# laurits-mumberg/kube-scheduler-simulator-p9

Hardware: AMD Instinct MI355X
Metric: filter+score pod x node pairs/sec (5k nodes, Fit+BalancedAllocation) (higher is better)
Workload: dtype int64+f64; 1 GPU; cfg2: 5,000 nodes x 10,000 pods, NodeResourcesFit+NodeResourcesBalancedAllocation; nodes_per_gpu=5000, nodes_total=5000, pods=10000, parallelism=1 GPU

## Files before the change

kube-scheduler-simulator-p9_amd/csrc/engine.hip:

```cpp
#include <hip/hip_runtime.h>

#include <algorithm>
#include <cmath>
#include <cstdlib>
#include <cstring>
#include <memory>
#include <string>
#include <vector>
#include <utility>
#include <deque>
#include <atomic>
#include <map>
#include <mutex>
#include <chrono>
#include <cstddef>
#include <thread>

#include "engine.h"
#include <rccl/rccl.h>

namespace ksg {

#define HIPCHK(x)                                                                 \
  do {                                                                            \
// ... 3319 lines not shown
    if (c == 0) {
      sm->feasible = feas;
      if (feas) {
        if (pt >= 0) {
          sm->max_score[pt] = max(red[0][0], red[1][0]) > sm->max_score[pt] ? max(red[0][0], red[1][0]) : sm->max_score[pt];
          sm->min_score[pt] = min(red[0][1], red[1][1]) < sm->min_score[pt] ? min(red[0][1], red[1][1]) : sm->min_score[pt];
        }
        if (pa >= 0) {
          sm->max_score[pa] = max(red[0][2], red[1][2]) > sm->max_score[pa] ? max(red[0][2], red[1][2]) : sm->max_score[pa];
          sm->min_score[pa] = min(red[0][3], red[1][3]) < sm->min_score[pa] ? min(red[0][3], red[1][3]) : sm->min_score[pa];
        }
      }
    }
    if (phase == 1) {
      A.wc_cls[(size_t)j * KSG_WC_CLS + c] = m;
      if (c == 0) A.wc_flag[j] = flag;
      return;
    }
    __syncthreads();
  } else {
    flag = A.wc_flag[j];
  }
  const bool kept = A.keep_n && q >= A.keep_first && q < A.keep_first + A.keep_n;
  if (kept) return;
  const int32_t feas_all = sm->feasible;
  const int64_t Mt = pt >= 0 ? sm->max_score[pt] : 0, Ma = pa >= 0 ? sm->max_score[pa] : 0;
  const int64_t wt = pt >= 0 ? F.weight[pt] : 0, wa = pa >= 0 ? F.weight[pa] : 0;
  bool range_err = false;
  uint64_t best = 0;
  if (present) {
    int64_t tot = (int64_t)(m >> 40);
    if (pt >= 0) {
      const int64_t s = Mt == 0 ? 100 : 100 - 100 * xt / Mt;
      range_err |= s < 0 || s > 100;
      tot += s * wt;
    }
    if (pa >= 0 && !(h->flags & KPF_SKIP_NA_SCORE)) {
      const int64_t s = Ma == 0 ? xa : 100 * xa / Ma;
      range_err |= s < 0 || s > 100;
      tot += s * wa;
    }
    if (feas_all == 1) tot = 0;
    best = ((uint64_t)tot << 40) | (m & 0xFFFFFFFFFFull);
  }
  best = wave_max(best);
  range_err = __ballot(range_err) != 0;
  if (lane == 0) {
    red[w][4] = (int64_t)best;
    red[w][5] = range_err ? 1 : 0;
  }
  __syncthreads();
  if (c == 0) {
    const uint64_t b = (uint64_t)red[0][4] > (uint64_t)red[1][4] ? (uint64_t)red[0][4] : (uint64_t)red[1][4];
    if (b) atomicMax((unsigned long long*)&sm->best_key, (unsigned long long)b);
    if (feas_all > 1 && (flag || red[0][5] || red[1][5])) atomicOr((uint32_t*)&sm->status, 2u);
  }
}

__device__ __forceinline__ int pend_index(int32_t gid, int32_t pn, int np) {
  int hit = -1;
  for (int e = 0; e < np; ++e) hit = __builtin_amdgcn_readlane(pn, e) == gid ? e : hit;
  return hit;
}
__device__ __forceinline__ void lds_barrier() { asm volatile("s_waitcnt lgkmcnt(0)\n\ts_barrier" ::: "memory"); }
__device__ __forceinline__ uint64_t ld_agent(const uint64_t* p) {
  return __hip_atomic_load(p, __ATOMIC_RELAXED, __HIP_MEMORY_SCOPE_AGENT);
}

struct PatchV {
  uint32_t code;
  int32_t fitba;
  int32_t total;
  uint32_t raw;
};
struct ShallowRows {
  RowV row[KSG_STAGE];
};
__device__ __forceinline__ ShallowRows* shallow_rows(uint8_t* rec) { return reinterpret_cast<ShallowRows*>(rec_rows(rec)); }
__device__ __forceinline__ const ShallowRows* shallow_rows(const uint8_t* rec) {
  return reinterpret_cast<const ShallowRows*>(rec_rows(rec));
}
static_assert(KSG_BATCH * sizeof(ShallowRows) <= kRecKeys * sizeof(RowV), "shallow rows fit the rows area");
static_assert(sizeof(ShallowRows) % 8 == 0, "8-byte words");
template <bool PER>
__device__ __forceinline__ void win_merge(const DevCluster& C, const WinArgs& A, uint32_t b, uint64_t* L, const int32_t* pnl,
                                          int np) {
  const int lane = threadIdx.x & 63, w = threadIdx.x >> 6;
  auto pend_lds = [&](int32_t gid) {
    int hit = -1;
    for (int e = 0; e < np; ++e) hit = pnl[e] == gid ? e : hit;
    return hit;
  };
  int32_t f[3] = {0, 0, 0};
  {
    const uint64_t* src = A.tile_top + (size_t)b * A.T * KSG_TOPK;
    uint64_t v = 0;
    if ((uint32_t)w < A.T) v = ld_agent(src + (size_t)w * KSG_TOPK + lane);
    if (w == 0)
      for (uint32_t t = lane; t < A.T; t += 64)
#pragma unroll
        for (int k = 0; k < 3; ++k)
          f[k] += __hip_atomic_load(A.tile_feas + ((size_t)b * A.T + t) * 3 + k, __ATOMIC_RELAXED, __HIP_MEMORY_SCOPE_AGENT);
#pragma unroll 1
    for (uint32_t t = w + 16; t < A.T; t += 16) v = wave_merge_top(v, ld_agent(src + (size_t)t * KSG_TOPK + 63 - lane));
    L[w * 64 + lane] = v;
  }
  lds_barrier();
  int s0 = 1;
  while (s0 < (int)A.T && s0 < 16) s0 <<= 1;
#pragma unroll 1
  for (int s = s0 >> 1; s >= 1; s >>= 1) {
    if (w < s) L[w * 64 + lane] = wave_merge_top(L[w * 64 + lane], L[(w + s) * 64 + 63 - lane]);
    lds_barrier();
  }
  if (w == 0) {
    const uint64_t v = L[lane];
    const int32_t gid = (int32_t)(v & 0xFFFFFull);
    stv<PER>(rec_keys(A.erec) + (size_t)b * KSG_CAND + lane, v);
    if (PER ? lane < KSG_STAGE : !A.xrows) {
      RowV c;
      memset(&c, 0, sizeof(c));
      if (v) {
        const int hh = pend_lds(gid);
        if (hh >= 0) c = ld_obj<PER>(&A.pprev[hh].after);
        else load_row_p<PER>(C, (uint32_t)gid - C.goff, A.need_eph, c);
      }
      st_obj<PER>(PER ? &shallow_rows(A.erec)[b].row[lane] : rec_rows(A.erec) + (size_t)b * KSG_CAND + lane, c);
    }
#pragma unroll
    for (int k = 0; k < 3; ++k) f[k] = wave_sum(f[k]);
    if (lane == 0) {
#pragma unroll
      for (int k = 0; k < 3; ++k) stv<PER>(reinterpret_cast<int32_t*>(A.erec) + k * KSG_BATCH + b, f[k]);
      stv<PER>(A.arrive + b * A.astride, 0u);
    }
    if constexpr (PER) {
      asm volatile("s_waitcnt vmcnt(0)" ::: "memory");
      if (lane == 0) __hip_atomic_fetch_add(A.evd, 1u, __ATOMIC_RELAXED, __HIP_MEMORY_SCOPE_AGENT);
    }
    if (lane == 0 && A.estamps) atomicMax((unsigned long long*)&A.estamps[10], (unsigned long long)__builtin_amdgcn_s_memrealtime());
  }
}
template <int MODE, bool STAT, bool PER = false>
__device__ __forceinline__ void win_eval(const DevCluster& C, const DevProfile& F, const WinArgs& A, uint32_t blk, uint64_t* L) {
  const int tid = threadIdx.x, lane = tid & 63, w = tid >> 6;
  uint32_t* wcount = reinterpret_cast<uint32_t*>(L + 16 * 64);
  const uint32_t b = blk / A.T, tile = blk - b * A.T, q = A.e0 + b;
  PodLite* h = reinterpret_cast<PodLite*>(wcount + 96);
  int64_t* mlds = reinterpret_cast<int64_t*>(wcount + 96 + sizeof(PodLite) / 4);
  RowV rnext;
  {
    const uint32_t nn0 = tile * A.tile_len + tid;
    if ((uint32_t)tid < A.tile_len && nn0 < C.N) load_row_p<PER>(C, nn0, A.need_eph, rnext);
  }
  {
    constexpr int kPodW = (int)(sizeof(PodLite) / 8);
    if (tid < kPodW) reinterpret_cast<uint64_t*>(h)[tid] = reinterpret_cast<const uint64_t*>(A.plite + q)[tid];
    if (STAT && tid < 2) mlds[tid] = ldv<PER>(A.mpred + 2 * (q - A.first) + tid);
  }
  const int np = ldv<PER>(A.pprev_n);
  int32_t* pnl = reinterpret_cast<int32_t*>(wcount + 64);
  if (tid < np) pnl[tid] = ldv<PER>(&A.pprev[tid].node);
  lds_barrier();
  auto pend_lds = [&](int32_t gid) {
    int hit = -1;
    for (int e = 0; e < np; ++e) hit = pnl[e] == gid ? e : hit;
    return hit;
  };
  const uint64_t t_start = A.estamps ? __builtin_amdgcn_s_memrealtime() : 0;
  if (A.estamps && tid == 0) {
    atomicMax((unsigned long long*)&A.estamps[8], ~(unsigned long long)t_start);
    atomicMax((unsigned long long*)&A.estamps[30], (unsigned long long)t_start);
  }
  uint64_t top = 0;
  uint32_t cF = 0, cT = 0, cA = 0;
  const bool est = A.estamps && tid == 960;
  uint64_t t_eval = 0, t_sort = 0, t_wait = 0;
#define KSG_ETIME(v)                             \
  __builtin_amdgcn_sched_barrier(0);         \
  const uint64_t v = __builtin_amdgcn_s_memtime(); \
  __builtin_amdgcn_sched_barrier(0);
  PatchV* stash = reinterpret_cast<PatchV*>(wcount + 192);
  const bool stash_all = A.npt <= A.stash_npt;
  static_assert(96 * 4 + sizeof(PodLite) + 16 <= 192 * 4, "eval LDS layout");
  auto fetch = [&](uint32_t kk, RowV& r, StaticRec& sr, bool loaded) {
    const uint32_t to = kk * KSG_TILE + tid, nn = tile * A.tile_len + to;
    if (to < A.tile_len && nn < C.N) {
      const int hit = pend_lds((int32_t)(C.goff + nn));
      if (hit >= 0) r = ld_obj<PER>(&A.pprev[hit].after);
      else if (!loaded) load_row_p<PER>(C, nn, A.need_eph, r);
      if (STAT) sr = srec_at<PER>(A, q, C.goff + nn);
    }
  };
  StaticRec snext{KSG_FILTER_PASS, 0};
  fetch(0, rnext, snext, true);
#pragma unroll 1
  for (uint32_t k = 0; k < A.npt; ++k) {
  KSG_ETIME(t0);
  if (A.estamps && w == 15) asm volatile("s_waitcnt vmcnt(0)" ::: "memory");
  KSG_ETIME(tl);
  t_wait += tl - t0;
  const uint32_t to = k * KSG_TILE + tid, n = tile * A.tile_len + to;
  const RowV r = rnext;
  const StaticRec sr = snext;
  if (k + 1 < A.npt) fetch(k + 1, rnext, snext, false);
  uint64_t key = 0;
  bool feasible = false, achT = false, achA = false;
  if (to < A.tile_len && n < C.N) {
    int32_t fit_s, ba_s;
    int64_t total;
    uint32_t code, raw = 0;
    if (STAT) {
      const int64_t MT = mlds[0], MA = mlds[1];
      code = eval_row_s<MODE>(r, F, h, C.R < 4 ? C.R : 4, sr, MT, MA, fit_s, ba_s, total);
      raw = sr.raw;
      achT = F.pos_taint >= 0 && (int64_t)(raw >> 20) == MT;
      achA = F.pos_na >= 0 && !(h->flags & KPF_SKIP_NA_SCORE) && (int64_t)(raw & KSG_RAW_NA_MASK) == MA;
    } else {
      code = eval_row<MODE>(r, F, h, C.R < 4 ? C.R : 4, fit_s, ba_s, total);
    }
    if (stash_all || w == 0) {
      stash[(stash_all ? k * 16 + w : k) * 64 + lane] = PatchV{code, fit_s | (ba_s << 16), (int32_t)total, raw};
    } else {
      uint32_t* of;
      int32_t *os, *ot;
      out_ptrs(A, q, C.N, of, os, ot);
      if (PER && kept_q(A, q)) write_pair<STAT, true>(F, of, os, ot, C.N, n, code, fit_s, ba_s, total, raw);
      else write_pair<STAT, false>(F, of, os, ot, C.N, n, code, fit_s, ba_s, total, raw);
    }
    if (code == KSG_FILTER_PASS) {
      feasible = true;
      key = pack_key(total, F.seed, h->queue_idx, C.goff + n);
    }
  }
  cF += (uint32_t)__popcll(__ballot(feasible));
  if (STAT) {
    cT += (uint32_t)__popcll(__ballot(feasible && achT));
    cA += (uint32_t)__popcll(__ballot(feasible && achA));
  }
  KSG_ETIME(t1);
  key = wave_sort_desc(key);
  top = k == 0 ? key : wave_merge_top(top, wave_reverse(key));
  KSG_ETIME(t2);
  t_eval += t1 - t0;
  t_sort += t2 - t1;
  }
  KSG_ETIME(t3);
  L[w * 64 + lane] = top;
  if (lane == 0) {
    wcount[w] = cF;
    wcount[32 + w] = cT;
    wcount[48 + w] = cA;
  }
  lds_barrier();
#pragma unroll 1
  for (int s = 8; s >= 1; s >>= 1) {
    if (w < s) L[w * 64 + lane] = wave_merge_top(L[w * 64 + lane], L[(w + s) * 64 + 63 - lane]);
    lds_barrier();
  }
  if (w == 0) {
    uint64_t* dst = A.tile_top + ((size_t)b * A.T + tile) * KSG_TOPK;
    __hip_atomic_store(dst + lane, L[lane], __ATOMIC_RELAXED, __HIP_MEMORY_SCOPE_AGENT);
    if (lane < 3) {
      const int off = lane == 0 ? 0 : 16 + 16 * lane;
      int32_t c = 0;
      for (int k = 0; k < 16; ++k) c += (int32_t)wcount[off + k];
      __hip_atomic_store(A.tile_feas + ((size_t)b * A.T + tile) * 3 + lane, c, __ATOMIC_RELAXED,
                         __HIP_MEMORY_SCOPE_AGENT);
    }
    asm volatile("s_waitcnt vmcnt(0)" ::: "memory");
    uint32_t old = 0;
    if (lane == 0) old = __hip_atomic_fetch_add(A.arrive + b * A.astride, 1u, __ATOMIC_RELAXED, __HIP_MEMORY_SCOPE_AGENT);
    old = __builtin_amdgcn_readfirstlane(old);
// ... 24 lines not shown
  KSG_ETIME(t4);
#undef KSG_ETIME
  if (est) {
    atomicAdd((unsigned long long*)&A.estamps[13], (unsigned long long)t_eval);
    atomicAdd((unsigned long long*)&A.estamps[14], (unsigned long long)t_sort);
    atomicAdd((unsigned long long*)&A.estamps[15], (unsigned long long)(t4 - t3));
    atomicAdd((unsigned long long*)&A.estamps[18], (unsigned long long)t_wait);
  }
  if (A.estamps && tid == 0) {
    __builtin_amdgcn_sched_barrier(0);
    const uint64_t t = __builtin_amdgcn_s_memrealtime();
    __builtin_amdgcn_sched_barrier(0);
    atomicMax((unsigned long long*)&A.estamps[9], (unsigned long long)t);
    atomicMax((unsigned long long*)&A.estamps[28], (unsigned long long)(t - t_start));
    atomicAdd((unsigned long long*)&A.estamps[29], (unsigned long long)(t - t_start));
    atomicAdd((unsigned long long*)&A.estamps[31], 1ull);
  }
  if (!wcount[16]) {
    flush_stash();
    signal_flushed();
    return;
  }
  win_merge<PER>(C, A, b, L, pnl, np);
  flush_stash();
  signal_flushed();
}

struct SumLite {
  uint64_t best_key;
  int32_t selected, feasible, status, pad;
};
struct Delta {
  int64_t req[4];
  int64_t nzc, nzm;
  int32_t pods;
};
#define KSG_HSLOTS 128
struct PickTab {
  int32_t node[KSG_HSLOTS];
  int32_t first[KSG_HSLOTS];
};
struct PickRow {
  RowV base;
  RowV after;
  RowV snap;
  int32_t node;
  int32_t nx;
  int32_t deep, pad;
};
struct WinLDS {
  uint64_t key[KSG_BATCH][KSG_CAND];
  RowV row[KSG_BATCH][KSG_STAGE];
  Pend prior[KSG_BATCH];
  PodLite pod[KSG_BATCH];
  PatchV patch[KSG_BATCH][KSG_CAND];
  uint64_t pkey[KSG_BATCH][KSG_BATCH];
  int8_t pdf[KSG_BATCH][KSG_BATCH];
  uint64_t pmask[KSG_BATCH];
  uint32_t nxt_ok;
  uint64_t pbest[KSG_BATCH];
  int32_t pbest_e[KSG_BATCH];
  int32_t S[3][KSG_BATCH];
  int32_t O[3][KSG_BATCH];
  int32_t feas[KSG_BATCH];
  SumLite sum[KSG_BATCH];
  int32_t ptn[KSG_HSLOTS], pte[KSG_HSLOTS];
  int32_t gtn[KSG_HSLOTS], gtf[KSG_HSLOTS];
  PickTab pick[3];
  PickRow pr[KSG_BATCH];
  uint64_t kc[KSG_BATCH][KSG_CAND];
  uint64_t rk[KSG_BATCH][KSG_BATCH];
  int8_t rdf[KSG_BATCH][KSG_BATCH];
  int32_t pf[KSG_BATCH];
  int32_t achT[KSG_BATCH], achA[KSG_BATCH];
  int64_t mt[KSG_BATCH], ma[KSG_BATCH];
  int64_t xmt[KSG_BATCH], xma[KSG_BATCH];
  int8_t pdfT[KSG_BATCH][KSG_BATCH], pdfA[KSG_BATCH][KSG_BATCH];
  int8_t rdfT[KSG_BATCH][KSG_BATCH], rdfA[KSG_BATCH][KSG_BATCH];
  int32_t fbf[KSG_BATCH];
  uint64_t red[16][4];
};

static_assert(sizeof(WinLDS) <= 160 * 1024, "window LDS exceeds the CU's 160 KiB");
static constexpr uint32_t kStashNpt =
    (uint32_t)std::min<size_t>(KSG_STASH_NPT, (sizeof(WinLDS) - (16 * 64 * 8 + 192 * 4)) / (16 * 64 * sizeof(PatchV)));
static_assert(kStashNpt >= 1, "eval blocks' output stash exceeds the window LDS");
__device__ __forceinline__ uint32_t hslot(int32_t node) { return ((uint32_t)node * 2654435761u) >> 25; }
__device__ __forceinline__ int prior_of(const WinLDS& L, int32_t x) {
  uint32_t h = hslot(x);
  for (int k = 0; k < KSG_HSLOTS; ++k) {
    int32_t v = L.ptn[h];
    if (v == x) return L.pte[h];
    if (v == -1) return -1;
    h = (h + 1) & (KSG_HSLOTS - 1);
  }
  return -1;
}
__device__ __forceinline__ uint32_t tab_claim(int32_t* nodes, int32_t x) {
  uint32_t h = hslot(x);
  for (int k = 0; k < KSG_HSLOTS; ++k) {
    int32_t old = atomicCAS(&nodes[h], -1, x);
    if (old == -1 || old == x) return h;
    h = (h + 1) & (KSG_HSLOTS - 1);
  }
  return 0;
}
__device__ __forceinline__ int tab_find(const int32_t* nodes, int32_t x) {
  uint32_t h = hslot(x);
  for (int k = 0; k < KSG_HSLOTS; ++k) {
    int32_t v = nodes[h];
    if (v == x) return (int)h;
    if (v == -1) return -1;
    h = (h + 1) & (KSG_HSLOTS - 1);
  }
  return -1;
}
__device__ __forceinline__ void pick_insert(PickTab& T, int32_t x, int b) {
  uint32_t h = tab_claim(T.node, x);
  atomicMin(&T.first[h], b);
}
__device__ __forceinline__ void pick_clear(PickTab& T, int i) {
  T.node[i] = -1;
  T.first[i] = KSG_BATCH;
}
__device__ __forceinline__ int first_pick(const PickTab& T, int32_t x) {
  int h = x >= 0 ? tab_find(T.node, x) : -1;
  return h >= 0 ? T.first[h] : KSG_BATCH;
}

#define KSG_ORG_NODE 0x40000000
template <bool PER = false>
__device__ __forceinline__ void origin_rows(const DevCluster& C, const WinLDS& L, const WinArgs& A, int32_t o,
                                            RowV& start, RowV& snap) {
  if (o & KSG_ORG_NODE) {
    if (A.xrows) start = A.xrows[o & 0xFFFFF];
    else load_row(C, (uint32_t)(o & 0xFFFFF) - C.goff, A.need_eph, start);
    snap = start;
  } else if (o < KSG_BATCH) {
    start = L.prior[o].after;
    snap = L.prior[o].base;
  } else {
    int p = (o - 64) >> 6, i = (o - 64) & 63;
    if (i < KSG_STAGE) start = L.row[p][i];
    else if (PER) load_row_p<PER>(C, (uint32_t)(L.key[p][i] & 0xFFFFFull) - C.goff, A.need_eph, start);
    else start = rec_rows(A.wrec)[p * KSG_CAND + i];
    snap = start;
  }
}
__device__ __forceinline__ void delta_of(const PodLite& p, Delta& d) {
#pragma unroll
  for (int k = 0; k < 4; ++k) d.req[k] = p.req[k];
  d.nzc = p.nz_cpu;
  d.nzm = p.nz_mem;
  d.pods = 1;
}
__device__ __forceinline__ void delta_add(Delta& d, const PodLite& p) {
#pragma unroll
  for (int k = 0; k < 4; ++k) d.req[k] += p.req[k];
  d.nzc += p.nz_cpu;
  d.nzm += p.nz_mem;
  d.pods += 1;
}
__device__ __forceinline__ void apply_delta(RowV& r, const Delta& d, uint32_t R) {
#pragma unroll
  for (uint32_t k = 0; k < 4; ++k)
    if (k < R) r.req[k] += d.req[k];
  r.nzc += d.nzc;
  r.nzm += d.nzm;
// ... 332 lines not shown
    const bool valid = b < nb;
    const uint64_t pm = valid ? L.pmask[b] : 0;
    const uint64_t pbk = valid ? L.pbest[b] : 0;
    int r = 0;
    bool pok = pbk != 0;
    int32_t node = -1, org = -1;
#pragma unroll 1
    for (int round = 0; round < 64; ++round) {
      uint64_t ck = 0;
      if (valid) {
        uint64_t free_ = ~pm & (r < 64 ? (~0ull << r) : 0ull);
        r = free_ ? __ffsll((long long)free_) - 1 : KSG_CAND;
        ck = r < KSG_CAND ? L.key[b][r] : 0;
      }
      uint64_t pk = pok ? pbk : 0;
      uint64_t best = ck > pk ? ck : pk;
      bool from_c = best != 0 && best == ck;
      node = best ? (int32_t)(best & 0xFFFFFull) : -1;
      org = !best ? -1 : from_c ? 64 + b * 64 + r : L.pbest_e[b];
      L.gtn[lane] = -1;
      L.gtn[lane + 64] = -1;
      uint32_t h = 0;
      if (node >= 0) {
        h = tab_claim(L.gtn, node);
        L.gtf[h] = KSG_BATCH;
      }
      if (node >= 0) atomicMin(&L.gtf[h], b);
      bool lose = node >= 0 && L.gtf[h] < b;
      if (__ballot(lose) == 0) break;
      if (lose) {
        if (from_c) ++r;
        else pok = false;
      }
    }
    if (lane < KSG_BATCH) {
      PickRow& e = L.pr[b];
      e.node = node;
      e.nx = KSG_BATCH;
      if (valid) {
        L.S[0][b] = node;
        L.O[0][b] = org;
      }
      const bool deep = node >= 0 && org >= 64 && ((org - 64) & 63) >= KSG_STAGE;
      e.deep = deep ? 1 : 0;
      if (node >= 0) pick_insert(L.pick[0], node, b);
      if (node >= 0 && !deep) {
        RowV st, snap;
        origin_rows<PER>(C, L, A, org, st, snap);
        e.base = st;
        e.snap = snap;
        Delta d;
        delta_of(L.pod[b], d);
        apply_delta(st, d, R);
        e.after = st;
      }
    }
  }
  lds_barrier();
  STAMP(3);
  int cur = 0, stable = 0;
  uint32_t iters = 0;
#pragma unroll 1
  for (;;) {
    const int nxt = cur == 2 ? 0 : cur + 1;
    if (tid < KSG_HSLOTS) pick_clear(L.pick[nxt == 2 ? 0 : nxt + 1], tid);
    const PickTab& T = L.pick[cur];
    if (wave < 8) {
      const int p_hi = nb * (nb - 1) / 2;
      if (iters == 0 && tid == 8 * 64 - 1 && L.pr[nb - 1].deep) {
        PickRow& e = L.pr[nb - 1];
        RowV st, snap;
        origin_rows<PER>(C, L, A, L.O[cur][nb - 1], st, snap);
        e.base = st;
        e.snap = snap;
        Delta d;
        delta_of(L.pod[nb - 1], d);
        apply_delta(st, d, R);
        e.after = st;
      }
#pragma unroll 1
      for (int base = stable * (stable - 1) / 2 + wave * 64; base < p_hi; base += 8 * 64) {
        const int p = base + lane;
        if (p < p_hi) {
          int b = (int)((1.0f + sqrtf(1.0f + 8.0f * (float)p)) * 0.5f);
          b = b * (b - 1) / 2 > p ? b - 1 : ((b + 1) * b / 2 <= p ? b + 1 : b);
          const int a = p - b * (b - 1) / 2;
          PickRow& e = L.pr[a];
          const int32_t Sv = e.node;
          uint64_t k = 0;
          int df = 0, dT = 0, dA = 0;
          PatchV pt;
          pt.code = KSG_NOT_PATCHED;
          pt.fitba = pt.total = 0;
          pt.raw = 0;
          if (Sv >= 0) {
            if (iters == 0) STAMP(24);
            const int nx = e.nx;
            if (iters == 0) STAMP(25);
            if (nx >= b) {
              RowV cur_r, snap;
              if (e.deep) {
                origin_rows<PER>(C, L, A, L.O[cur][a], cur_r, snap);
                if (b == a + 1) {
                  e.base = cur_r;
                  e.snap = snap;
                }
                Delta d;
                delta_of(L.pod[a], d);
                apply_delta(cur_r, d, R);
                if (b == a + 1) e.after = cur_r;
              } else {
                cur_r = e.after;
                snap = e.snap;
              }
              const PodLite* h = &L.pod[b];
              int32_t fs, bs;
              int64_t tot;

              StaticRec sr{KSG_FILTER_PASS, 0};
              uint32_t code;
              if (STAT) {
                sr = srec_at<PER>(A, A.w0 + b, (uint32_t)Sv);
                code = eval_row_s<MODE>(cur_r, F, h, R, sr, L.mt[b], L.ma[b], fs, bs, tot);
              } else {
                code = eval_row<MODE>(cur_r, F, h, R, fs, bs, tot);
              }

              bool snap_ok = sr.code == KSG_FILTER_PASS && (F.pos_fit < 0 || fit_filter_row(snap, h, R) == 0);
              df = (code == KSG_FILTER_PASS ? 1 : 0) - (snap_ok ? 1 : 0);
              if (STAT) {
                const bool na_on = F.pos_na >= 0 && !(h->flags & KPF_SKIP_NA_SCORE);
                dT = F.pos_taint >= 0 && (int64_t)(sr.raw >> 20) == L.mt[b] ? df : 0;
                dA = na_on && (int64_t)(sr.raw & KSG_RAW_NA_MASK) == L.ma[b] ? df : 0;
              }
              if (code == KSG_FILTER_PASS) k = pack_key(tot, F.seed, h->queue_idx, (uint32_t)Sv);
              pt.code = code;
              pt.fitba = fs | (bs << 16);
              pt.total = (int32_t)tot;
              pt.raw = sr.raw;
            }
          }
          L.rk[b][a] = k;
          L.rdf[b][a] = (int8_t)df;
          if (STAT) {
            L.rdfT[b][a] = (int8_t)dT;
            L.rdfA[b][a] = (int8_t)dA;
          }
          L.patch[b][32 + a] = pt;
        }
      }
    } else {
      if (wave == 8 && lane < np) L.pf[lane] = first_pick(T, L.prior[lane].node);
#pragma unroll 1
      for (int b = stable + (wave - 8); b < nb; b += 8) {
        const uint64_t ck = L.key[b][lane];
        const bool mod = ((L.pmask[b] >> lane) & 1) || (ck != 0 && first_pick(T, (int32_t)(ck & 0xFFFFFull)) < b);
        L.kc[b][lane] = mod ? 0 : ck;
      }
    }
    if (iters == 0) STAMP(21);
    lds_barrier();
    if (iters == 0) STAMP(22);
    if constexpr (STAT) {
#pragma unroll 1
      for (int hh = 0; hh < 2; ++hh) {
        const int b = 2 * wave + hh;
        if (b >= nb) break;
// ... 91 lines not shown
          {
            const bool perr = (fl & KPF_PREFILTER_ERROR) != 0 || na_prescore_error(fl, feasible);
            const int32_t sel = (feasible > 0 && bk && !perr) ? (int32_t)(bk & 0xFFFFFull) : -1;
            int32_t org = -1;
            if (c) org = 64 + b * 64 + (__ffsll((long long)c) - 1);
            else if (p) org = __ffsll((long long)p) - 1;
            else if (r) org = L.O[cur][__ffsll((long long)r) - 1];
            L.S[nxt][b] = sel;
            L.O[nxt][b] = sel >= 0 ? org : -1;
            if (sel >= 0) pick_insert(L.pick[nxt], sel, b);
            SumLite& sm = L.sum[b];
            sm.best_key = sel >= 0 ? (feasible == 1 ? (bk & 0xFFFFFFFFFFull) : bk) : 0;
            sm.selected = sel;
            sm.feasible = feasible;
            sm.status = perr ? 2 : (sel >= 0 ? 0 : 1);
          }
        }
      }
    }
    if (iters == 0) STAMP(23);
    lds_barrier();
    if (STAT) {
      unsigned long long fm = __ballot(lane < nb && lane >= stable && L.fbf[lane & 31] != 0);
      if (fm) {
        while (fm) {
          const int b = __ffsll((long long)fm) - 1;
          fm &= fm - 1;
          win_exact_select<MODE, PER>(C, F, A, L, b, cur, nxt, R);
        }
        lds_barrier();
      }
    }
    if (iters < 2) STAMP(19 + iters);
    ++iters;
    bool changed;
    {
      const int32_t so = L.S[cur][lane & 31], sn = L.S[nxt][lane & 31];
      unsigned long long m = __ballot(lane < nb && lane >= stable && sn != so);
      stable = m ? min(__ffsll((long long)m), nb) : nb;
      changed = m != 0;
    }
    cur = nxt;
    if (!changed) break;
    win_fill_rows<PER>(C, L, A, L.S[cur], L.O[cur], nb, stable, R, tid);
    lds_barrier();
    if (stable >= nb) break;
  }
  STAMP(4);
  if (A.stamps && tid == 0) A.stamps[7] = iters;
  uint32_t pre_fl = 0, pre_ev = 0;
  if (PER && tid == 0) {
    pre_fl = ld_sc1(A.flushed);
    pre_ev = A.nxt_evd ? ld_sc1(A.nxt_evd) : 0u;
  }
  auto flushed_wait = [&]() {
    if (tid == 0) {
      bool ok = pre_fl >= A.flush_need;
      for (uint32_t it = 0; !ok && it < A.spin; ++it) {
        if (ld_sc1(A.flushed) >= A.flush_need) { ok = true; break; }
        if ((it & 63u) == 63u && ld_sc1(A.abortw) != 0u) break;
        __builtin_amdgcn_s_sleep(2);
      }
      if (!ok) __hip_atomic_store(A.abortw, 1u, __ATOMIC_RELAXED, __HIP_MEMORY_SCOPE_AGENT);
    }
    lds_barrier();
  };
  auto exact_writes = [&]() {
    unsigned long long fm = __ballot(lane < nb && L.fbf[lane & 31] != 0);
    while (fm) {
      const int b = __ffsll((long long)fm) - 1;
      fm &= fm - 1;
      win_exact_write<MODE, PER>(C, F, A, L, b, cur, R);
    }
  };
  bool exact_early = false;
  if constexpr (PER && STAT) {
    if (A.replay2 && __ballot(lane < nb && L.fbf[lane & 31] != 0) != 0) {
      exact_early = true;
      flushed_wait();
      exact_writes();
    }
  }
  const PickTab& T = L.pick[cur];
  if (wave == 0) {
    const int a = lane;
    const PickRow& e = L.pr[a & 31];
    const bool last = a < nb && e.node >= 0 && e.nx == KSG_BATCH;
    unsigned long long m = __ballot(last);
    if (last) {
      Pend p;
      p.node = e.node;
      p.pad = 0;
      p.base = e.base;
      p.after = e.after;
      st_obj<PER>(A.pnext + __popcll(m & ((1ull << a) - 1)), p);
    }
    if (lane == 0) stv<PER>(A.pnext_n, (int32_t)__popcll(m));
  }
  STAMP(26);
  if constexpr (PER) {
    asm volatile("s_waitcnt vmcnt(0)" ::: "memory");
    STAMP(27);
    __syncthreads();
    if (tid < 16) {
      if (A.replay2) __hip_atomic_fetch_max(A.pub + tid * 32, A.pub_val, __ATOMIC_RELAXED, __HIP_MEMORY_SCOPE_AGENT);
      else st_sc1(A.pub + tid * 32, A.pub_val);
    }
    if (A.rstamps && tid == 0) A.rstamps[2] = __builtin_amdgcn_s_memrealtime();
  }
  STAMP(6);
  if (tid < nb) {
    ksg_pod_summary& d = A.sums[A.w0 + tid];
    d.best_key = L.sum[tid].best_key;
    d.selected = L.sum[tid].selected;
    d.feasible = L.sum[tid].feasible;
    d.status = L.sum[tid].status;
    if (STAT) {
      if (F.pos_taint >= 0) d.max_score[F.pos_taint] = L.xmt[tid];
      if (F.pos_na >= 0) d.max_score[F.pos_na] = L.xma[tid];
    }
  }
  if constexpr (PER) {
    if (tid == 0) L.nxt_ok = A.nxt_evd && pre_ev >= A.nxt_need ? 1u : 0u;
    if (!exact_early) flushed_wait();
  }
  {
    const int32_t Sv = L.S[cur][lane & 31];
    const int32_t pn = lane < np ? L.prior[lane].node : -1;
    const int pf = lane < np ? first_pick(T, pn) : -1;
#pragma unroll 1
    for (int hh = 0; hh < 2; ++hh) {
      const int b = 2 * wave + hh;
      if (b >= nb) break;
      if (STAT && L.fbf[b]) continue;
      const PatchV pt = L.patch[b][lane];
      const bool wr = lane < 32 ? (lane < np && pf >= b) : (lane - 32 < b && pt.code != KSG_NOT_PATCHED);
      const int32_t node = lane < 32 ? pn : Sv;
      const uint32_t nl = (uint32_t)node - C.goff;
      if (wr && node >= 0 && (uint32_t)node >= C.goff && nl < C.N) {
        uint32_t* of;
        int32_t *os, *ot;
        out_ptrs(A, A.w0 + b, C.N, of, os, ot);
        if (PER && kept_q(A, A.w0 + b))
          write_pair<STAT, true>(F, of, os, ot, C.N, nl, pt.code, pt.fitba & 0xFFFF, pt.fitba >> 16, pt.total, pt.raw);
        else
          write_pair<STAT, false>(F, of, os, ot, C.N, nl, pt.code, pt.fitba & 0xFFFF, pt.fitba >> 16, pt.total, pt.raw);
      }
    }
  }
  if (STAT && !exact_early) exact_writes();
  STAMP(5);
  if (A.stamps && tid == 0) A.stamps[12] = __builtin_amdgcn_s_memrealtime();
#undef STAMP
}

template <int MODE, bool STAT>
__global__ __launch_bounds__(KSG_WIN_THREADS) void k_window(DevCluster C, DevProfile F, WinArgs A) {
  extern __shared__ __attribute__((aligned(16))) unsigned char lds_raw[];
  uint32_t warm = 0;
  KWarm<0, (int)((sizeof(DevCluster) + sizeof(DevProfile) + sizeof(WinArgs)) / 64 * 64)>::run(
      (const void*)__builtin_amdgcn_kernarg_segment_ptr(), warm);
  warm_wait(warm);
  if (blockIdx.x == 0) {
    if (A.nw) win_fixup<MODE, STAT>(C, F, A, *reinterpret_cast<WinLDS*>(lds_raw));
    return;
  }
  win_eval<MODE, STAT>(C, F, A, blockIdx.x - 1, reinterpret_cast<uint64_t*>(lds_raw));
// ... 1149 lines not shown
                          uint32_t* arrive = nullptr) -> bool {
    const uint32_t q0 = first + c * chunk, cn = std::min(chunk, first + count - q0);
    if (!ready)
      HIPCHK(hipMemsetAsync(I.mpred.p + 2 * (size_t)(q0 - first), 0xFF, 2 * (size_t)cn * sizeof(int64_t), st));
    const dim3 sgrid(std::max<uint32_t>((SN + 256 * KSG_ST_NPT - 1) / (256 * KSG_ST_NPT), 1),
                     (cn + KSG_ST_PODS - 1) / KSG_ST_PODS);
    const bool ssamp = I.sample_every && (st == s || ready);
    if (ssamp) {
      while (I.sev_st.size() < 2 * (size_t)(I.n_st + 1)) {
        hipEvent_t e;
        HIPCHK(hipEventCreate(&e));
        I.sev_st.push_back(e);
      }
      HIPCHK(hipEventRecord(I.sev_st[2 * I.n_st], st));
    }
    StaticRec* const sout = I.stat.p + (size_t)((q0 - first) % (nslots * chunk)) * A.stat_n;
    const bool dec = static_dec_ok(q0, cn);
    if (ready && !dec) { err = "static records beside the loop: pods that do not decode"; return false; }
    if (dec) {
      if (!I.sd_pods.alloc((size_t)chunk * (sizeof(WcPod) / 8), err)) return false;
      WcPod* wp = reinterpret_cast<WcPod*>(I.sd_pods.p);
      hipLaunchKernelGGL(k_st_decode, dim3((cn + 63) / 64), dim3(64), 0, st, CS, I.F, I.progs.p, I.prog_off_d.p, q0, cn,
                         wp, gstat ? 1 : 0);
      const dim3 dgrid(std::max<uint32_t>((SN + 256 * KSG_SD_NPT - 1) / (256 * KSG_SD_NPT), 1),
                       (cn + KSG_SD_PODS - 1) / KSG_SD_PODS);
      if (run_grid) {
        const uint32_t ntx = std::max<uint32_t>((SN + 1024 * KSG_SD_NPT - 1) / (1024 * KSG_SD_NPT), 1);
        const uint32_t items = ntx * ((cn + KSG_SD_PODS - 1) / KSG_SD_PODS);
        hipLaunchKernelGGL(k_static_dec_run, dim3(std::min(run_grid, items)), dim3(1024), 0, st, CS, I.F, wp, I.progs.p, cn,
                           sout, I.mpred.p + 2 * (size_t)(q0 - first), ready, ntx, items, arrive);
      } else {
        hipLaunchKernelGGL(k_static_dec, dgrid, dim3(256), 0, st, CS, I.F, wp, I.progs.p, cn, sout,
                           I.mpred.p + 2 * (size_t)(q0 - first), ready);
      }
      I.static_dec_chunks++;
    } else {
      hipLaunchKernelGGL(k_static, sgrid, dim3(256), 0, st, CS, I.F, I.progs.p, I.prog_off_d.p, q0, cn, sout,
                         I.mpred.p + 2 * (size_t)(q0 - first), gstat ? 1 : 0);
    }
    if (ssamp) {
      HIPCHK(hipEventRecord(I.sev_st[2 * I.n_st + 1], st));
      I.stat_pods_sampled += cn;
      I.n_st++;
    }
    return true;
  };
  if (sharded && !stat) return run_batches_split(I, A, first, count, T, err);
  if (persist_ok && (!stat || stat_run)) {
    const bool r2 = (stat ? I.win_replay2_stat : I.win_replay2) && 2 + (uint64_t)KSG_BATCH * T <= I.n_cus;
    const uint32_t nrep = r2 ? 2u : 1u;
    const uint32_t grid = nrep + KSG_BATCH * T;
    const uint32_t side_grid = I.n_cus > grid ? I.n_cus - grid : 0;
    const bool overlap = stat_run && I.static_overlap && I.sstream && side_grid > 0 && static_dec_ok(first, count);
    const uint32_t sgroups = (count + KSG_SD_PODS - 1) / KSG_SD_PODS;
    uint32_t side_blocks = 0;
    auto issue_side = [&]() -> bool {
      if (!issue_static(0, I.sstream, I.sready.p, side_grid, I.sready.p + sgroups)) return false;
      HIPCHK(hipEventRecord(I.sev_ready, I.sstream));
      return true;
    };
    if (overlap) {
      const uint32_t ntx = std::max<uint32_t>((SN + 1024 * KSG_SD_NPT - 1) / (1024 * KSG_SD_NPT), 1);
      side_blocks = std::min<uint32_t>(side_grid, ntx * sgroups);
      if (!I.sready.alloc(sgroups + 1, err) || !I.sd_pods.alloc((size_t)chunk * (sizeof(WcPod) / 8), err)) return false;
      HIPCHK(hipMemsetAsync(I.sready.p, 0, (sgroups + 1) * sizeof(uint32_t), s));
      HIPCHK(hipMemsetAsync(I.mpred.p, 0xFF, 2 * (size_t)count * sizeof(int64_t), s));
      if (!I.sev_ready)
        for (auto* e : {&I.sev_ready, &I.sev_free})
          HIPCHK(hipEventCreateWithFlags(e, hipEventDisableTiming));
      HIPCHK(hipEventRecord(I.sev_free, s));
      HIPCHK(hipStreamWaitEvent(I.sstream, I.sev_free, 0));
      if (I.static_beside_test == 0 && !issue_side()) return false;
    } else if (stat_run && !issue_static(0, s)) {
      return false;
    }
    if (!I.wsync.alloc(1, err) || !I.rsync.alloc(1, err)) return false;
    if (!I.hverdict) {
      HIPCHK(hipHostMalloc((void**)&I.hverdict, kVerdictBytes, hipHostMallocCoherent | hipHostMallocMapped));
      HIPCHK(hipMemsetAsync(I.rsync.p, 0, sizeof(RunSync), s));
    }
    HIPCHK(hipMemsetAsync(I.wsync.p, 0, sizeof(WinSync), s));
    HIPCHK(hipMemsetAsync(I.rsync.p, 0, kRunSyncReset, s));
    HIPCHK(hipMemsetAsync(I.arrive.p, 0, 2 * KSG_BATCH * 32 * sizeof(uint32_t), s));
    WinRunArgs R{};
    R.nwin = nwin;
    R.first = first;
    R.count = count;
    R.T = T;
    R.tt_sz = (uint32_t)tt_sz;
    R.tf_sz = (uint32_t)tf_sz;
    R.tile_top = I.tile_top.p;
    R.tfeas = I.tfeas.p;
    R.wrec = I.wrec.p;
    R.pend = I.pend.p;
    R.pend_n = I.pend_n.p;
    R.arrive = I.arrive.p;
    R.stamps = I.stamps_on ? I.stamps.p : nullptr;
    R.sready = overlap ? I.sready.p : nullptr;
    R.sready_need = std::max<uint32_t>((SN + 1024 * KSG_SD_NPT - 1) / (1024 * KSG_SD_NPT), 1);
    WinArgs AP = A;
    AP.astride = 32;
    AP.replay2 = r2 ? 1u : 0u;
    __atomic_store_n(I.hverdict, 0u, __ATOMIC_RELEASE);
    RunCtl RC{grid + I.run_need_extra, I.run_wait_us * 100u, 0, I.hverdict, I.run_spin};
    if (overlap) {
      RC.side_arrive = I.sready.p + sgroups;
      RC.side_need = side_blocks;
    }
    bool sampled;
    if (!sample_begin(I, s, true, sampled, err)) return false;
    hipLaunchKernelGGL(kWindowRun[stat_run][I.eval_mode == 1], dim3(grid), dim3(KSG_WIN_THREADS), sizeof(WinLDS), s, C, I.F, AP, R,
                       I.rsync.p, I.wsync.p, RC);
    if (!sample_end(I, s, sampled, err)) return false;
    HIPCHK(hipGetLastError());
    if (overlap && I.static_beside_test == 1 && !issue_side()) return false;
    I.run_used = true;
    const uint32_t v = wait_verdict(I, s, err);
    if (overlap && I.static_beside_test == 2 && !issue_side()) return false;
    if (v == 0u) return false;
    if (v == 3u) {
      I.lost = true;
      err = "persistent launch: a gate never completed (blocks not co-resident?)";
      return false;
    }
    if (v == 1u) {
      I.win_runs++;
      if (overlap) {
        HIPCHK(hipStreamWaitEvent(s, I.sev_ready, 0));
        I.static_overlaps++;
      }
      const int64_t L = nwin - 1;
      hipLaunchKernelGGL(k_apply_pend, dim3(1), dim3(KSG_BATCH), 0, s, C, I.pend.p + (size_t)(L & 1) * KSG_BATCH,
                         I.pend_n.p + (L & 1));
      HIPCHK(hipEventRecord(I.ev1, s));
      HIPCHK(hipGetLastError());
      return true;
    }
    I.win_fallbacks++;
    if (sampled) I.n_samples--;
    if (overlap) HIPCHK(hipStreamWaitEvent(s, I.sev_ready, 0));
  }
  for (int64_t j = -1; j < (int64_t)nwin; ++j) {
    const int64_t E = j + 1, W = j;
    A.ne = 0;
    A.nw = 0;
    A.stamps = A.estamps = nullptr;
    A.tile_top = I.tile_top.p + (size_t)(E & 1) * tt_sz;
    A.tile_feas = I.tfeas.p + (size_t)(E & 1) * tf_sz;
    if (E < (int64_t)nwin) {
      A.estamps = I.stamps_on ? I.stamps.p + (size_t)E * 32 : nullptr;
      A.e0 = first + (uint32_t)E * KSG_BATCH;
      A.ne = std::min<uint32_t>(KSG_BATCH, first + count - A.e0);
      A.erec = sharded ? I.xsend.p : I.wrec.p + (size_t)(E & 1) * kRecBytes;
    }
    if (W >= 0) {
      A.w0 = first + (uint32_t)W * KSG_BATCH;
      A.nw = std::min<uint32_t>(KSG_BATCH, first + count - A.w0);
      A.wrec = I.wrec.p + (size_t)(W & 1) * kRecBytes;
      A.pnext = I.pend.p + (size_t)(W & 1) * KSG_BATCH;
      A.pnext_n = I.pend_n.p + (W & 1);
      A.stamps = I.stamps_on ? I.stamps.p + (size_t)W * 32 : nullptr;
    }
    const int64_t P = W - 1;
    A.pprev = I.pend.p + (size_t)(P & 1) * KSG_BATCH;
    A.pprev_n = I.pend_n.p + (P & 1);
    const bool chunk_start = stat && A.ne && (A.e0 - first) % chunk == 0;
// ... 1935 lines not shown
```

Baseline: 8.814 billion pairs/s.

## Stage previous-window pending rows in LDS and write pend list word-parallel

In the persistent path, eval blocks now load the previous window's pending-node list as a fixed batch of 64-bit words spread across threads. The 'after' rows are cached in LDS, so per-node fetches read LDS instead of global memory. The count load is dropped, and unused slots carry a -1 sentinel, which the host initialises by memsetting the pend buffer. The writer side stores the pend entries one word per thread across the whole block instead of from a single wave, and the stash area shrinks to make room. A fast sqrt builtin replaces sqrtf in the pair index decode. The cost is a smaller output stash and reliance on the sentinel invariant.

```diff
diff --git a/kube-scheduler-simulator-p9_amd/csrc/engine.hip b/kube-scheduler-simulator-p9_amd/csrc/engine.hip
--- a/kube-scheduler-simulator-p9_amd/csrc/engine.hip
+++ b/kube-scheduler-simulator-p9_amd/csrc/engine.hip
@@ -3425,6 +3425,8 @@
 }
 static_assert(KSG_BATCH * sizeof(ShallowRows) <= kRecKeys * sizeof(RowV), "shallow rows fit the rows area");
 static_assert(sizeof(ShallowRows) % 8 == 0, "8-byte words");
+constexpr size_t kEvalRowArea = KSG_BATCH * sizeof(RowV);
+static_assert(kEvalRowArea % 16 == 0, "the stash behind it holds 16-byte entries");
 template <bool PER>
 __device__ __forceinline__ void win_merge(const DevCluster& C, const WinArgs& A, uint32_t b, uint64_t* L, const int32_t* pnl,
                                           int np) {
@@ -3501,9 +3503,25 @@
     if (tid < kPodW) reinterpret_cast<uint64_t*>(h)[tid] = reinterpret_cast<const uint64_t*>(A.plite + q)[tid];
     if (STAT && tid < 2) mlds[tid] = ldv<PER>(A.mpred + 2 * (q - A.first) + tid);
   }
-  const int np = ldv<PER>(A.pprev_n);
   int32_t* pnl = reinterpret_cast<int32_t*>(wcount + 64);
-  if (tid < np) pnl[tid] = ldv<PER>(&A.pprev[tid].node);
+  uint64_t* const rarea = reinterpret_cast<uint64_t*>(wcount + 192);
+  int np;
+  if constexpr (PER) {
+    constexpr int kRowW = (int)(sizeof(RowV) / 8), kPendW = (int)(sizeof(Pend) / 8);
+    static_assert(offsetof(Pend, node) == 0 && offsetof(Pend, after) == (size_t)(kPendW - kRowW) * 8, "Pend words");
+    static_assert(KSG_BATCH * (kRowW + 1) <= KSG_WIN_THREADS, "one word of P_{E-2} per thread");
+    np = KSG_BATCH;
+    if (tid < KSG_BATCH * (kRowW + 1)) {
+      const int e = tid / (kRowW + 1), k = tid - e * (kRowW + 1);
+      const uint64_t* pe = reinterpret_cast<const uint64_t*>(A.pprev + e);
+      const uint64_t v = ld_sc1(pe + (k == 0 ? 0 : kPendW - kRowW + k - 1));
+      if (k == 0) pnl[e] = (int32_t)(uint32_t)v;
+      else rarea[e * kRowW + k - 1] = v;
+    }
+  } else {
+    np = ldv<PER>(A.pprev_n);
+    if (tid < np) pnl[tid] = ldv<PER>(&A.pprev[tid].node);
+  }
   lds_barrier();
   auto pend_lds = [&](int32_t gid) {
     int hit = -1;
@@ -3523,15 +3541,20 @@
   __builtin_amdgcn_sched_barrier(0);         \
   const uint64_t v = __builtin_amdgcn_s_memtime(); \
   __builtin_amdgcn_sched_barrier(0);
-  PatchV* stash = reinterpret_cast<PatchV*>(wcount + 192);
+  PatchV* stash = reinterpret_cast<PatchV*>(wcount + 192 + kEvalRowArea / 4);
   const bool stash_all = A.npt <= A.stash_npt;
   static_assert(96 * 4 + sizeof(PodLite) + 16 <= 192 * 4, "eval LDS layout");
+  static_assert((16 * 64 * 8 + 192 * 4) % 16 == 0, "row area and stash alignment");
   auto fetch = [&](uint32_t kk, RowV& r, StaticRec& sr, bool loaded) {
     const uint32_t to = kk * KSG_TILE + tid, nn = tile * A.tile_len + to;
     if (to < A.tile_len && nn < C.N) {
       const int hit = pend_lds((int32_t)(C.goff + nn));
-      if (hit >= 0) r = ld_obj<PER>(&A.pprev[hit].after);
-      else if (!loaded) load_row_p<PER>(C, nn, A.need_eph, r);
+      if constexpr (PER) {
+        if (hit >= 0) r = *reinterpret_cast<const RowV*>(rarea + hit * (int)(sizeof(RowV) / 8));
+      } else {
+        if (hit >= 0) r = ld_obj<PER>(&A.pprev[hit].after);
+      }
+      if (hit < 0 && !loaded) load_row_p<PER>(C, nn, A.need_eph, r);
       if (STAT) sr = srec_at<PER>(A, q, C.goff + nn);
     }
   };
@@ -3722,8 +3745,8 @@
 };
 
 static_assert(sizeof(WinLDS) <= 160 * 1024, "window LDS exceeds the CU's 160 KiB");
-static constexpr uint32_t kStashNpt =
-    (uint32_t)std::min<size_t>(KSG_STASH_NPT, (sizeof(WinLDS) - (16 * 64 * 8 + 192 * 4)) / (16 * 64 * sizeof(PatchV)));
+static constexpr uint32_t kStashNpt = (uint32_t)std::min<size_t>(
+    KSG_STASH_NPT, (sizeof(WinLDS) - (16 * 64 * 8 + 192 * 4 + kEvalRowArea)) / (16 * 64 * sizeof(PatchV)));
 static_assert(kStashNpt >= 1, "eval blocks' output stash exceeds the window LDS");
 __device__ __forceinline__ uint32_t hslot(int32_t node) { return ((uint32_t)node * 2654435761u) >> 25; }
 __device__ __forceinline__ int prior_of(const WinLDS& L, int32_t x) {
@@ -4222,7 +4245,7 @@
       for (int base = stable * (stable - 1) / 2 + wave * 64; base < p_hi; base += 8 * 64) {
         const int p = base + lane;
         if (p < p_hi) {
-          int b = (int)((1.0f + sqrtf(1.0f + 8.0f * (float)p)) * 0.5f);
+          int b = (int)((1.0f + __builtin_amdgcn_sqrtf(1.0f + 8.0f * (float)p)) * 0.5f);
           b = b * (b - 1) / 2 > p ? b - 1 : ((b + 1) * b / 2 <= p ? b + 1 : b);
           const int a = p - b * (b - 1) / 2;
           PickRow& e = L.pr[a];
@@ -4480,7 +4503,22 @@
     }
   }
   const PickTab& T = L.pick[cur];
-  if (wave == 0) {
+  if constexpr (PER) {
+    static_assert(offsetof(PickRow, base) == 0 && offsetof(PickRow, after) == sizeof(RowV), "PickRow: base, after first");
+    static_assert(offsetof(Pend, base) == 8 && offsetof(Pend, after) == 8 + sizeof(RowV), "Pend: node word, base, after");
+    static_assert(KSG_BATCH * kPendW <= KSG_WIN_THREADS, "one word of P_W per thread");
+    const PickRow& e = L.pr[lane & 31];
+    const uint32_t m = (uint32_t)__ballot(lane < nb && e.node >= 0 && e.nx == KSG_BATCH);
+    const int n = __popc(m);
+    const int a = tid / kPendW, k = tid - a * kPendW;
+    if (a < KSG_BATCH && ((m >> a) & 1u)) {
+      const PickRow& src = L.pr[a];
+      const uint64_t v = k == 0 ? (uint64_t)(uint32_t)src.node : reinterpret_cast<const uint64_t*>(&src)[k - 1];
+      st_sc1(reinterpret_cast<uint64_t*>(A.pnext + __popc(m & ((1u << a) - 1u))) + k, v);
+    }
+    if (tid < KSG_BATCH && tid >= n) st_sc1(reinterpret_cast<uint64_t*>(A.pnext + tid), 0xFFFFFFFFull);
+    if (tid == 0) st_sc1(A.pnext_n, (int32_t)n);
+  } else if (wave == 0) {
     const int a = lane;
     const PickRow& e = L.pr[a & 31];
     const bool last = a < nb && e.node >= 0 && e.nx == KSG_BATCH;
@@ -5796,6 +5834,7 @@
     HIPCHK(hipMemsetAsync(I.wsync.p, 0, sizeof(WinSync), s));
     HIPCHK(hipMemsetAsync(I.rsync.p, 0, kRunSyncReset, s));
     HIPCHK(hipMemsetAsync(I.arrive.p, 0, 2 * KSG_BATCH * 32 * sizeof(uint32_t), s));
+    HIPCHK(hipMemsetAsync(I.pend.p, 0xFF, 2 * KSG_BATCH * sizeof(Pend), s));
     WinRunArgs R{};
     R.nwin = nwin;
     R.first = first;
```

New measurement: 9.363 billion pairs/s (median of 6 runs). +6.2%, better.
